# koszullab/chromosight

Hardware: AMD Instinct MI355X
Metric: Mpixels/s normxcorr2 (17x17 loops kernel) (higher is better)
Workload: dtype f32

## Files before the change

chromosight_amd/csrc/cs_corr_mfma.hip:

```cpp
#include "cs_device.h"
#include <algorithm>
#include <cstdlib>
#include <cstring>
#include <mutex>
#include <utility>
#include <vector>

#include "cs_launch.h"

namespace cs {

typedef _Float16 h8 __attribute__((ext_vector_type(8)));

__device__ __forceinline__ float cand_range_guard(float r, float s2, float unscale, const KernelStats<float>& K);
typedef _Float16 h4 __attribute__((ext_vector_type(4)));
typedef float f4 __attribute__((ext_vector_type(4)));
typedef float f4u __attribute__((ext_vector_type(4), aligned(4)));
typedef double d2u __attribute__((ext_vector_type(2), aligned(8)));

constexpr int MF_T = 64;
constexpr int MF_R = 80;
constexpr int MF_PLANE = MF_R * MF_R * 2;
constexpr int MF_WSET = 17 * 2 * 1024;
constexpr int MF_SCR_PITCH = 40;
// ... 226 lines not shown

    load_set(0);
    __syncthreads();
    MF_STAMP(3);
    for (int s = 0; s < km; ++s) {
        const h8 bh = reinterpret_cast<const h8*>(wreg)[(2 * s + 0) * 64 + lane];
        const h8 bl = reinterpret_cast<const h8*>(wreg)[(2 * s + 1) * 64 + lane];
#pragma unroll
        for (int c = 0; c < 4; ++c) {
            const int off = (wr0 + s + n) * MF_R + 16 * c + 8 * g;
            const h8 ah = *reinterpret_cast<const h8*>(xh + off);
            const h8 al = *reinterpret_cast<const h8*>(xl + off);
            accM[c] = mfma16(ah, bh, accM[c]);
            accC[c] = mfma16(ah, bl, accC[c]);
            accC[c] = mfma16(al, bh, accC[c]);
        }
    }
    MF_STAMP(4);
    if constexpr (MASKED) {
        for (int set = 1; set <= 2; ++set) {
            __syncthreads();
            load_set(set);
            __syncthreads();
            for (int s = 0; s < km; ++s) {
                const h8 bh = reinterpret_cast<const h8*>(wreg)[(2 * s + 0) * 64 + lane];
                const h8 bl = reinterpret_cast<const h8*>(wreg)[(2 * s + 1) * 64 + lane];
#pragma unroll
                for (int c = 0; c < 4; ++c) {
                    const int off = (wr0 + s + n) * MF_R + 16 * c + 8 * g;
                    const h8 am = *reinterpret_cast<const h8*>(xm + off);
                    if (set == 1) {
                        KA[c] = mfma16(am, bh, KA[c]);
                        KA[c] = mfma16(am, bl, KA[c]);
                    } else {
                        KB[c] = mfma16(am, bh, KB[c]);
                        KB[c] = mfma16(am, bl, KB[c]);
                    }
                }
            }
        }
    }

    MF_STAMP(5);
    const float u_cs = unscale * E.unscale[0];
    const float u_s2 = 32.0f * unscale;
#pragma unroll
    for (int c = 0; c < 4; ++c) {
        const int j = J0 + 16 * c + n;
#pragma unroll
        for (int v = 0; v < 4; ++v) {
            const int i = I0 + wr0 + 4 * g + v;
            if (i >= A.row_end || j < 0 || j >= A.ns) continue;
            const int d = j - i;
            if (d < A.out_lo || d > A.out_hi) continue;
            const float cs = (accM[c][v] + accC[c][v]) * u_cs;
            const float s1 = S1[c][v] * unscale;
            const float s2 = (S2[c][v] * u_s2) * unscale;
            float r, nobs = A.ks.n;
            if (pixel_forced_zero(A, i, j)) {
                r = 0.0f;
            } else if (A.xcorr_only) {
                r = (fabsf(cs) < A.ks.thr) ? 0.0f : cs;
            } else if constexpr (MASKED) {
                const float nm = NM[c][v];
                const float ka = KA[c][v] * E.unscale[1], kb = KB[c][v] * E.unscale[2];
                r = cand_range_guard(pearson_masked_lean(cs, s1, s2, nm, ka, kb, A.ks), s2, unscale, A.ks);
                nobs = A.ks.n - nm;
            } else {
                r = cand_range_guard(pearson_nomask_lean(cs, s1, s2, A.ks), s2, unscale, A.ks);
            }
            store_pixel(A, i, j, r, nobs);
        }
    }
    MF_STAMP(6);
}

#ifdef CS_MF_PROFILE
extern "C" int cs_debug_mfma_profile(unsigned long long* out)
{
    hipError_t e = hipMemcpyFromSymbol(out, HIP_SYMBOL(cs_mf_prof), sizeof(cs_mf_prof));
    if (e != hipSuccess) return (int)e;
    unsigned long long zero[16] = {0};
    return (int)hipMemcpyToSymbol(HIP_SYMBOL(cs_mf_prof), zero, sizeof(zero));
}
#endif

struct MfmaFixArgs {
    int fix_on, fix_hi_w, fix_hi_d0;
    const float* fix_lo;
    const float* fix_hi;
    const float* fix_rows;
    const float* fix_cols;
    int fix_top, fix_bot0, fix_width, fix_xband, fix_xlo, fix_side;
    const float* rim;
    int max_dist;
};

struct MfmaDenseArgs {
    const float* sig;
    void* out;
    int out_is_f64;
    long long ld_in, ld_out, row0_in, row0_out;
    int ms, ns, km, kn;
    int row_begin, row_end;
    int full, sym_upper;
    int xcorr_only;
    int tiles_x, n_tiles;
    int by_cut;
    const uint4* frag;
    float w_unscale;
    float wa_unscale, wb_unscale;
    int xcd_order;
    int dbg;
    KernelStats<float> ks;
    int band_in, lo_in, bw_in;
    int pad_in;
    int cnt_in;
    int band_out, lo_out;
    int out_lo, out_hi;
    float* nobs;
    const float* w;
    const uint8_t* miss_col;
    const float* rowtab;
    const float* coltab;
    int fix_on, fix_hi_w, fix_hi_d0, fix_top, fix_bot0, fix_any_side;
    int rim_in_kernel;
    MfmaFixArgs fx;
};

constexpr int MFD_ROWS_PER_THREAD = 14;
constexpr int MFD_WL = 4 * MF_PLANE;
constexpr int MFD_SCR = MFD_WL + 18 * 1024;
constexpr int MFD_RED = MFD_SCR + 4 * 2 * MF_SCR_PLANE;
constexpr int MFD_SMEM = MFD_RED + 64;
constexpr int MFD_COL = MFD_RED + 64;
constexpr int MFD_CFL = MFD_COL + 2 * 3 * 64 * 4;
constexpr int MFD_CFB = MFD_CFL + 2 * 16;
constexpr int MFD_SMEM_REG = MFD_CFB + 2 * 128;
static_assert(MFD_SMEM_REG <= 80 * 1024, "two workgroups per CU");
#ifdef CS_MF_PROFILE
constexpr int MFD_PROF = MFD_SMEM_REG;
constexpr int MFD_LAUNCH_EXTRA = 128;
#else
constexpr int MFD_LAUNCH_EXTRA = 0;
#endif

__device__ __forceinline__ unsigned pack_h2(_Float16 a, _Float16 b)
{
    typedef _Float16 h2 __attribute__((ext_vector_type(2)));
    h2 v;
    v[0] = a;
    v[1] = b;
    return __builtin_bit_cast(unsigned, v);
}

__device__ __forceinline__ void lds_barrier()
{
    __builtin_amdgcn_fence(__ATOMIC_RELEASE, "workgroup", "local");
    __builtin_amdgcn_s_waitcnt(0xc07f);
    __builtin_amdgcn_s_barrier();
    __builtin_amdgcn_fence(__ATOMIC_ACQUIRE, "workgroup", "local");
}

__device__ __forceinline__ float wave_max_nonneg(float v)
{
#define CS_DPP_MAX(ctrl, rmask)                                                                                  \
    v = fmaxf(v, __builtin_bit_cast(float, __builtin_amdgcn_update_dpp(0, __builtin_bit_cast(int, v), ctrl, rmask, 0xf, true)))
    CS_DPP_MAX(0x111, 0xf);
    CS_DPP_MAX(0x112, 0xf);
    CS_DPP_MAX(0x114, 0xf);
    CS_DPP_MAX(0x118, 0xf);
    CS_DPP_MAX(0x142, 0xa);
    CS_DPP_MAX(0x143, 0xc);
#undef CS_DPP_MAX
    return v;
}

__device__ __forceinline__ void wave_lds_sync()
{
    __builtin_amdgcn_fence(__ATOMIC_RELEASE, "wavefront");
    __builtin_amdgcn_wave_barrier();
    __builtin_amdgcn_fence(__ATOMIC_ACQUIRE, "wavefront");
}

__device__ __forceinline__ float cand_range_guard(float r, float s2, float unscale, const KernelStats<float>& K)
{
    if (K.cand_cmin > 0.0f) r = ((int)(s2 > 0.0f) & (int)(s2 < K.n * (unscale * unscale) * 0.0625f)) ? 2.0f : r;
    return r;
}

__device__ __attribute__((noinline)) float masked_coefficient_rare(float cs, float s1, float s2, float nm, float ka, float kb,
                                                                   const KernelStats<float>& K)
{
    return pearson_masked_f32(cs, s1, s2, nm, ka, kb, K);
}

__device__ __forceinline__ float masked_coefficient(float cs, float s1, float s2, float nm, float ka, float kb,
                                                    const KernelStats<float>& K)
{
    bool rare;
    float r = pearson_masked_core(cs, s1, s2, nm, ka, kb, K, rare);
    if (rare) r = masked_coefficient_rare(cs, s1, s2, nm, ka, kb, K);
    return r;
}

typedef const __attribute__((address_space(4))) MfmaFixArgs* FixArgsPtr;

__device__ __forceinline__ FixArgsPtr fix_args()
{
    unsigned long long kv = (unsigned long long)__builtin_amdgcn_kernarg_segment_ptr();
    asm volatile("" : "+s"(kv));
    return (FixArgsPtr)(kv + offsetof(MfmaDenseArgs, fx));
}

typedef const __attribute__((address_space(4))) KernelStats<float>* StatsPtr;

__device__ __forceinline__ StatsPtr stats_args()
{
    unsigned long long kv = (unsigned long long)__builtin_amdgcn_kernarg_segment_ptr();
    asm volatile("" : "+s"(kv));
    return (StatsPtr)(kv + offsetof(MfmaDenseArgs, ks));
}

typedef const __attribute__((address_space(4))) MfmaDenseArgs* ArgsPtr;

__device__ __forceinline__ ArgsPtr args_here()
{
    unsigned long long kv = (unsigned long long)__builtin_amdgcn_kernarg_segment_ptr();
    asm volatile("" : "+s"(kv));
    return (ArgsPtr)kv;
}

typedef const __attribute__((address_space(4))) CountsHeader* CountsHdrPtr;

__device__ __forceinline__ CountsHdrPtr counts_header(const float* band)
{
    return (CountsHdrPtr)((unsigned long long)band - (unsigned long long)kCountsHeaderBytes);
}

__device__ __forceinline__ ArgsPtr args_at(unsigned long long entry)
{
    asm volatile("" : "+s"(entry));
    return (ArgsPtr)entry;
}

__device__ __forceinline__ FixArgsPtr fix_args_at(unsigned long long entry)
{
    asm volatile("" : "+s"(entry));
    return (FixArgsPtr)(entry + offsetof(MfmaDenseArgs, fx));
}

__device__ __forceinline__ StatsPtr stats_args_at(unsigned long long entry)
{
    asm volatile("" : "+s"(entry));
    return (StatsPtr)(entry + offsetof(MfmaDenseArgs, ks));
}

template <typename AT>
__device__ __forceinline__ const float* mask_fix_record(AT& A, FixArgsPtr F, int i, int j)
{
    const int K = A.km, KH = (A.km - 1) / 2;
    const int d = j - i;
    const int fix_on = F->fix_on, fix_side = F->fix_side, fix_top = F->fix_top, fix_bot0 = F->fix_bot0, fix_hi_d0 = F->fix_hi_d0,
              fix_hi_w = F->fix_hi_w;
    const float* fix_cols = F->fix_cols;
    const bool in_range = (j >= 0) & (j < A.ns) & (d >= A.out_lo) & (d <= A.out_hi) & (i < A.row_end);
    const int x = F->fix_xband ? d - F->fix_xlo : j;
    const bool top = i < fix_top;
    const bool bot = (i >= fix_bot0) & (!fix_on | (i + KH >= A.ms) | (j + KH >= A.ns));
    const bool side = (fix_cols != nullptr) & ((j < fix_side) | (j >= A.ns - fix_side));
    const bool edge_rec = (fix_on != 0) & (A.rim_in_kernel == 0);
    const bool lo = edge_rec & (d >= 0) & (d < K - 1);
    const bool hi = edge_rec & (d >= fix_hi_d0) & (d - fix_hi_d0 < fix_hi_w);
    const long long o_rows = (long long)(top ? i : fix_top + i - fix_bot0) * F->fix_width + x;
    const long long o_side = (long long)i * 2 * fix_side + (j < fix_side ? j : j - (A.ns - 2 * fix_side));
    const long long o_lo = (long long)i * (K - 1) + d;
    const long long o_hi = (long long)i * fix_hi_w + (d - fix_hi_d0);
    const float* base = (top | bot) ? F->fix_rows : side ? fix_cols : lo ? F->fix_lo : F->fix_hi;
    const long long off = (top | bot) ? o_rows : side ? o_side : lo ? o_lo : o_hi;
    return (in_range & (top | bot | side | lo | hi)) ? base + 4 * off : nullptr;
}

__device__ __forceinline__ void rim_correction(const float* __restrict__ T, int K, int D, int md, unsigned rbits, unsigned cbits,
                                               float& fn, float& fa, float& fb)
{
    fn = fa = fb = 0.0f;
    if (D < K - 1) {
        fn = T[kRimBase + D];
        fa = T[kRimBase + 17 + D];
        fb = T[kRimBase + 34 + D];
    }
    for (unsigned rb = rbits; rb; rb &= rb - 1) {
        const int ki = __builtin_ctz(rb);
        const int L = min(K, max(0, ki - D));
        const int H = min(K, max(0, md - D + ki + 1));
        const float* pa = T + kRimPW + ki * 18;
        const float* pb = pa + 17 * 18;
        fn -= (float)(L + (K - H));
        fa -= pa[L] + (pa[K] - pa[H]);
        fb -= pb[L] + (pb[K] - pb[H]);
    }
    for (unsigned cb = cbits; cb; cb &= cb - 1) {
        const int kj = __builtin_ctz(cb);
        const int lo_k = min(K, max(0, kj + D + 1));
        const int hi_k = min(K, max(0, kj - (md - D)));
        const float* qa = T + kRimQW + kj * 18;
// ... 381 lines not shown
```

chromosight_amd/csrc/cs_corr_mfma_body.inc:

```

    extern __shared__ __attribute__((aligned(16))) char smem[];
    char* const pl_xh = smem;
    char* const pl_xl = smem + MF_PLANE;
    char* const pl_qh = smem + 2 * MF_PLANE;
    char* const pl_ql = smem + 3 * MF_PLANE;
    float* const raw = reinterpret_cast<float*>(smem + 2 * MF_PLANE);
    const int tid = threadIdx.x;
    const int lane = tid & 63, wv = tid >> 6;
    const int n = lane & 15, g = lane >> 4;
    char* const scr = smem + MFD_SCR + wv * (2 * MF_SCR_PLANE);
    unsigned* const red = reinterpret_cast<unsigned*>(smem + MFD_RED);
    const int km = A.km, kn = A.kn;
    const int kh = (km - 1) / 2, kw = (kn - 1) / 2;
#ifdef CS_MF_PROFILE
#undef MF_PROF_ADD
#define MF_PROF_ADD(k, v) (prof_lds[k] += (unsigned long long)(v))
    unsigned long long* const prof_lds = reinterpret_cast<unsigned long long*>(smem + MFD_PROF);
    unsigned long long tprev_ = 0;
    if (tid == 0)
        for (int k = 0; k < 16; ++k) prof_lds[k] = 0;
    auto prof_flush = [&]() {
        if (tid == 0)
            for (int k = 0; k < 16; ++k)
                if (prof_lds[k]) atomicAdd(&cs_mf_prof[k], prof_lds[k]);
    };
#endif

    h8 ones_b, ones_p;
#pragma unroll
    for (int e = 0; e < 8; ++e) {
        const int t = 8 * g + e - n;
        ones_b[e] = (t >= 0 && t < kn) ? (_Float16)1.0f : (_Float16)0.0f;
        const int rho = (e < 4 ? 4 * g + e : 16 + 4 * g + (e - 4)) - n;
        ones_p[e] = (rho >= 0 && rho < km) ? (_Float16)1.0f : (_Float16)0.0f;
    }
    const f4 zero4 = {0.0f, 0.0f, 0.0f, 0.0f};
    const int wr0 = 16 * wv;
    const int c2 = tid % 40, rg = tid / 40;
    const int c2_ = c2, rg_ = rg;
    const bool stager = tid < 240;
    const int p_min = max(0, A.row_begin - kh), p_max = min(A.ms, A.row_end + (km - 1) - kh) - 1;
    int pad_row0 = 0x7fffffff;
    if constexpr (REG && VEC4) pad_row0 = A.pad_in ? max(p_min, (int)A.row0_in + 1) : 0x7fffffff;
    float cnt_max = 0.0f;
    const float* cnt_wt = nullptr;
    const float* cnt_rlaw = nullptr;
    int cnt_n = 1, cnt_nd = 1;
    if constexpr (REG && VEC4) {
        if (A.cnt_in) {
            const CountsHdrPtr H = counts_header(A.sig);
            cnt_max = (float)H->max_val;
            cnt_wt = H->weight32;
            cnt_rlaw = H->rlaw32;
            cnt_n = H->n;
            cnt_nd = H->n_diags;
        }
    }

    auto tile_origin = [&](int tile, int& I0, int& J0) {
        if constexpr (LIST) tile = tile_list[tile];
        int by = tile / A.tiles_x;
        int bx = tile - by * A.tiles_x;
        if constexpr (REG) {
            if (by >= A.by_cut) {
                int t = tile - A.by_cut * A.tiles_x;
                by = A.by_cut;
                for (;;) {
                    const int left = A.ns - (A.row_begin + by * MF_T + A.out_lo);
                    const int v = min(A.tiles_x, left <= 0 ? 0 : (left + MF_T - 1) / MF_T);
                    if (t < v) break;
                    t -= v;
                    ++by;
                }
                bx = t;
            }
        }
        I0 = A.row_begin + by * MF_T;
        if constexpr (!REG) {
            const int skew = A.xcd_order >> 1;
            if (skew) {
                bx += (by * skew) % A.tiles_x;
                bx -= bx >= A.tiles_x ? A.tiles_x : 0;
            }
        }
        J0 = bx * MF_T;
        if (REG && A.band_out) J0 += I0 + A.out_lo;
    };
    const int wv_u = __builtin_amdgcn_readfirstlane(wv);
    auto fetch_args = [&]() {
        if constexpr (REG) return TABLE ? args_at(table_entry) : args_here();
        else return &A;
    };
    constexpr int kPiecesPerRow = VEC4 ? MF_R / 4 : MF_R;
    constexpr int kTransfers = VEC4 ? 25 : 100;
    auto fetch = [&](int tile, int slot) {
        const auto FA = fetch_args();
        int I0, J0;
        tile_origin(tile, I0, J0);
        const int P0 = I0 - kh, Q0 = J0 - kw;
        const bool pad_tile = REG && VEC4 && P0 >= pad_row0 && P0 + MF_R - 1 <= p_max;
        int lane_f = lane;
        if constexpr (REG) asm volatile("" : "+v"(lane_f));
        const int e0 = 64 * wv_u + lane_f;
        int r = e0 / kPiecesPerRow, c = e0 - r * kPiecesPerRow;
        if (REG && !MFD_DBG(16384)) {
            if (wv_u < 3) {
                const float* src = FA->coltab + (size_t)wv_u * FA->ns + min(max(J0 + lane_f, 0), FA->ns - 1);
                __builtin_amdgcn_global_load_lds(src, (__attribute__((address_space(3))) void*)(
                    (__attribute__((address_space(3))) char*)(smem) + MFD_COL + (slot * 3 + wv_u) * 256), 4, 0, 0);
            } else {
                const long long base = (long long)(uintptr_t)FA->miss_col;
                const long long first = ((base + Q0) >> 2) << 2;
                long long addr = first + 4 * min(lane_f, 23);
                addr = min(max(addr, (base >> 2) << 2), ((base + FA->ns - 1) >> 2) << 2);
                if (lane_f < 24)
                    __builtin_amdgcn_global_load_lds(reinterpret_cast<const unsigned*>((uintptr_t)addr),
                                                     (__attribute__((address_space(3))) void*)(
                                                         (__attribute__((address_space(3))) char*)(smem) + MFD_CFB + slot * 128), 4, 0, 0);
            }
        }
        if constexpr (REG && VEC4) {
            if (FA->cnt_in) {
                const float* wt = cnt_wt;
                const float* rlaw = cnt_rlaw;
                const int hn = cnt_n, hd = cnt_nd;
#pragma unroll 1
                for (int x = wv_u; x < 5; x += 4) {
                    const int e = 64 * x + lane_f;
                    const bool is_w = e < 160;
                    const int idx = e < 80 ? P0 + e : e < 160 ? Q0 + (e - 80) : Q0 - P0 - (MF_R - 1) + (e - 160);
                    const float* src = (is_w ? wt : rlaw) + min(max(idx, is_w ? 0 : -1), is_w ? hn - 1 : hd);
                    __builtin_amdgcn_global_load_lds(src, (__attribute__((address_space(3))) void*)(
                                                              (__attribute__((address_space(3))) char*)(smem) + MFD_SCR + 256 * x), 4, 0, 0);
                }
            }
        }
        const __attribute__((address_space(3))) char* dst =
            (const __attribute__((address_space(3))) char*)(raw) + (VEC4 ? 1024 : 256) * wv_u;
        if constexpr (REG && VEC4) {
            if (FA->band_in && P0 >= p_min && P0 + MF_R - 1 <= p_max && Q0 - (P0 + MF_R - 1) - FA->lo_in >= 0 &&
                Q0 + MF_R - 1 - P0 - FA->lo_in <= FA->bw_in - 1) {
                const float* src = FA->sig + ((long long)P0 - FA->row0_in) * FA->ld_in + (Q0 - P0 - FA->lo_in) + (long long)r * (FA->ld_in - 1) + 4 * c;
                const long long step_r = 12 * (FA->ld_in - 1) + 64, wrap = (FA->ld_in - 1) - 80;
#pragma unroll 1
                for (int i = wv_u; i < kTransfers; i += 4) {
                    __builtin_amdgcn_global_load_lds(src, (__attribute__((address_space(3))) void*)dst, 16, 0, 0);
                    dst += 4096;
                    c += 16;
                    src += step_r;
                    if (c >= kPiecesPerRow) {
                        c -= kPiecesPerRow;
                        src += wrap;
                    }
                }
                return;
            }
        }
#pragma unroll 1
        for (int i = wv_u; i < kTransfers; i += 4) {
            const int p = min(max(P0 + r, p_min), p_max);
            const float* row = FA->sig + ((long long)p - FA->row0_in) * FA->ld_in;
            if constexpr (VEC4) {
                int q = Q0 + 4 * c;
                if (REG && FA->band_in) q = pad_tile ? min(max(q - p - FA->lo_in, -4), FA->bw_in) : min(max(q - p - FA->lo_in, 0), FA->bw_in - 4);
                else q = min(max(q, 0), FA->ns - 4);
                __builtin_amdgcn_global_load_lds(row + q, (__attribute__((address_space(3))) void*)dst, 16, 0, 0);
                dst += 4096;
                c += 256 % kPiecesPerRow;
                r += 256 / kPiecesPerRow;
            } else {
                int q = min(max(Q0 + c, 0), FA->ns - 1);
                if (REG && FA->band_in) q = min(max(q - p - FA->lo_in, 0), FA->bw_in - 1);
                __builtin_amdgcn_global_load_lds(row + q, (__attribute__((address_space(3))) void*)dst, 4, 0, 0);
                dst += 1024;
                c += 256 % kPiecesPerRow;
                r += 256 / kPiecesPerRow;
            }
            if (c >= kPiecesPerRow) {
                c -= kPiecesPerRow;
                r += 1;
            }
        }
    };

    auto emit = [&](int I0, int J0, float unscale, const f4 (&acc)[4], const f4 (&S1)[4], const f4 (&S2)[4],
                    const f4& hdr, int slot) {
        const float u_cs = unscale * A.w_unscale;
        const float u_s2 = 32.0f * unscale;
        if constexpr (REG) {
            const ArgsPtr EA = TABLE ? args_at(table_entry) : args_here();
            const int K = km;
            const int i = I0 + wr0 + n;
            KernelStats<float> KS;
            {
                const StatsPtr sp = TABLE ? stats_args_at(table_entry) : stats_args();
                KS.n = sp->n; KS.inv_n = sp->inv_n; KS.kmean = sp->kmean; KS.kstd = sp->kstd; KS.kvar = sp->kvar;
                KS.ksum = sp->ksum; KS.k2sum = sp->k2sum; KS.thr = sp->thr; KS.eps = sp->eps; KS.cut = sp->cut;
                KS.thr_n = sp->thr_n; KS.nkvar = sp->nkvar; KS.eps2 = sp->eps2; KS.den2_min = sp->den2_min;
                KS.zk_possible = sp->zk_possible; KS.snap_possible = sp->snap_possible;
                KS.cand_cmin = CAND ? sp->cand_cmin : 0.0f;
                KS.cand_thr = CAND ? sp->cand_thr : 0.0f;
            }
            const float* colb = reinterpret_cast<const float*>(smem + MFD_COL) + slot * 3 * 64;
            const float nr = hdr[0], ra = hdr[1], rb = hdr[2];
            const unsigned* cfm = reinterpret_cast<const unsigned*>(smem + MFD_CFL) + slot * 4;
            const unsigned m0 = __builtin_amdgcn_readfirstlane(cfm[0]), m1 = __builtin_amdgcn_readfirstlane(cfm[1]),
                           m2 = __builtin_amdgcn_readfirstlane(cfm[2]);
            const bool tile_flags = (m0 | m1 | m2) != 0;
            const unsigned row_bits = (tile_flags && !MFD_DBG(128)) ? (unsigned)hdr[3] : 0u;
            const bool cross_on = __builtin_amdgcn_ballot_w64(row_bits != 0) != 0;
            h8 ua_h, ua_t, ub_h, ub_t;
            if (cross_on) {
                float ua[8], ub[8];
#pragma unroll
                for (int e = 0; e < 8; ++e) ua[e] = ub[e] = 0.0f;
                unsigned bits = row_bits;
                while (__builtin_amdgcn_ballot_w64(bits != 0)) {
                    if (bits) {
                        const int ki = __builtin_ctz(bits);
                        bits &= bits - 1;
                        const float* wa = EA->w + K * K + ki * K;
                        const float* wb = EA->w + 2 * K * K + ki * K;
#pragma unroll
                        for (int e = 0; e < 8; ++e) {
                            const int kj = 8 * g + e;
                            const float in = kj < K ? 1.0f : 0.0f;
                            ua[e] = fmaf(wa[min(kj, K - 1)], in, ua[e]);
                            ub[e] = fmaf(wb[min(kj, K - 1)], in, ub[e]);
                        }
                    }
                }
                const float sa = __builtin_amdgcn_rcpf(EA->wa_unscale), sb = __builtin_amdgcn_rcpf(EA->wb_unscale);
#pragma unroll
                for (int e = 0; e < 8; ++e) {
                    const float a = ua[e] * sa, b = ub[e] * sb;
                    ua_h[e] = (_Float16)a;
                    ua_t[e] = (_Float16)(a - (float)ua_h[e]);
                    ub_h[e] = (_Float16)b;
                    ub_t[e] = (_Float16)(b - (float)ub_h[e]);
                }
            }
            MF_STAMP(7);
            const unsigned kmask8 = (((1u << K) - 1u) >> (8 * g)) & 0xffu;
            const int dmin = J0 - (I0 + MF_T - 1), dmax = J0 + MF_T - 1 - I0;
            const bool on_edge_diag = EA->fix_on && ((dmin < K - 1 && dmax >= 0) | (dmax >= EA->fix_hi_d0 && dmin < EA->fix_hi_d0 + EA->fix_hi_w));
            const bool right_or_bottom = !EA->fix_on | (I0 + MF_T - 1 + (K - 1) / 2 >= EA->ms) | (J0 + MF_T - 1 + (K - 1) / 2 >= EA->ns);
            const bool needs_fix = !MFD_DBG(256) && ((I0 < EA->fix_top) | ((I0 + MF_T - 1 >= EA->fix_bot0) & right_or_bottom) | (EA->fix_any_side != 0) |
                                   (on_edge_diag && !EA->rim_in_kernel));
            const bool needs_rim = RSYM && !MFD_DBG(256) && on_edge_diag && EA->rim_in_kernel;
            const bool plain_out = I0 + MF_T <= EA->row_end && J0 >= 0 && J0 + MF_T <= EA->ns && dmin >= EA->out_lo && dmax <= EA->out_hi;
            float* tb = reinterpret_cast<float*>(scr);
            const bool tile_forced = EA->sym_upper && dmin + (kn - km) < 0;
            f4 fxn = zero4, fxa = zero4, fxb = zero4;
            unsigned fxc = 0xffffu;
            if constexpr (RSYM) if (needs_rim) {
                const FixArgsPtr F = TABLE ? fix_args_at(table_entry) : fix_args();
                const int hi_d0 = F->fix_hi_d0, hi_w = F->fix_hi_w;
                const int iw0 = I0 + wr0;
                const int wd_lo = J0 - iw0 - 15, wd_hi = J0 + MF_T - 1 - iw0;
                const bool low = wd_lo < K - 1 && wd_hi >= 0;
                const bool up = wd_hi >= hi_d0 && wd_lo < hi_d0 + hi_w;
                if (low | up) {
                    const float* rimtab = F->rim;
                    const int md = F->max_dist, bot0 = F->fix_bot0;
                    const int KHf = (K - 1) / 2;
                    const int d0 = low ? 0 : hi_d0, dn = low ? K - 1 : hi_w;
                    const int a = i + d0 - J0;
                    const unsigned rb_all = (unsigned)hdr[3];
                    const bool row_ok = (i >= KHf) & (i + KHf < EA->ms) & (i < EA->row_end);
                    fxc = 0u;
#pragma unroll
                    for (int v = 0; v < 4; ++v) {
                        const int c = (a - 4 * g - v + 15) >> 4;
                        const int x = 16 * c + 4 * g + v;
                        const int d = d0 + (x - a), j = J0 + x;
                        const bool framed = (i >= bot0) & ((i + KHf >= EA->ms) | (j + KHf >= EA->ns));
                        const bool on = row_ok & (c >= 0) & (c <= 3) & (x - a < dn) & !framed & (j >= KHf) & (j + KHf < EA->ns) &
                                        (d >= EA->out_lo) & (d <= EA->out_hi);
                        float fn = 0.0f, fa = 0.0f, fb = 0.0f;
                        if (on) {
                            const unsigned lo32 = x < 32 ? m0 : x < 64 ? m1 : m2;
                            const unsigned hi32 = x < 32 ? m1 : x < 64 ? m2 : 0u;
                            const unsigned cb = (unsigned)((((unsigned long long)hi32 << 32) | lo32) >> (x & 31)) & ((1u << K) - 1u);
                            rim_correction(rimtab, K, d, md, rb_all, cb, fn, fa, fb);
                        }
                        fxn[v] = fn;
                        fxa[v] = fa;
                        fxb[v] = fb;
                        fxc |= (on ? (unsigned)c : 15u) << (4 * v);
                    }
                }
// ... 109 lines not shown
                        }
                        bool live = s2 > 0.0f;
                        if (tile_forced) {
                            const bool forced = d + (kn - km) < 0;
                            if (forced) val = 0.0f;
                            live &= !forced;
                        }
                        if (!plain_out) live &= (i < EA->row_end) & (j >= 0) & (j < EA->ns) & (d >= EA->out_lo) & (d <= EA->out_hi);
                        if (rare && live) rare_bits |= 1u << (4 * cc + v);
                        rv[cc][v] = val;
                    }
                }
#pragma unroll 1
                for (int k = 0; k < (CAND ? 0 : 8); ++k) {
                    if (!__builtin_amdgcn_ballot_w64((rare_bits >> k) != 0)) break;
                    if ((rare_bits >> k) & 1u) {
                        float cs = 0.0f, s1 = 0.0f, s2 = 0.0f, nm = 0.0f, ka = 0.0f, kb = 0.0f;
#pragma unroll
                        for (int e = 0; e < 8; ++e) {
                            const int c = 2 * half + (e >> 2), v = e & 3;
                            if (e == k) {
                                cs = acc[c][v] * u_cs;
                                s1 = S1[c][v] * unscale;
                                s2 = (S2[c][v] * u_s2) * unscale;
                                nm = nmv[e >> 2][v];
                                ka = kav[e >> 2][v];
                                kb = kbv[e >> 2][v];
                            }
                        }
                        const float val = pearson_masked_f32(cs, s1, s2, nm, ka, kb, KS);
#pragma unroll
                        for (int e = 0; e < 8; ++e)
                            if (e == k) rv[e >> 2][e & 3] = val;
                    }
                }
                MF_STAMP(10);
                if constexpr (CAND) {
                    unsigned long long* keys = reinterpret_cast<unsigned long long*>(EA->out);
                    unsigned long long* counter = reinterpret_cast<unsigned long long*>(EA->nobs);
                    float top = rv[0][0];
#pragma unroll
                    for (int e = 1; e < 8; ++e) top = fmaxf(top, rv[e >> 2][e & 3]);
                    if (!__builtin_amdgcn_ballot_w64(top >= KS.cand_thr)) continue;
#pragma unroll
                    for (int cc = 0; cc < 2; ++cc) {
#pragma unroll
                        for (int v = 0; v < 4; ++v) {
                            const int j = J0 + 16 * (2 * half + cc) + 4 * g + v;
                            const int d = j - i;
                            const bool hit = (rv[cc][v] >= KS.cand_thr) & (i < EA->row_end) & (j >= 0) & (j < EA->ns) &
                                             (d >= EA->out_lo) & (d <= EA->out_hi);
                            const unsigned long long m = __builtin_amdgcn_ballot_w64(hit);
                            if (m) {
                                const int first = __builtin_ctzll(m);
                                unsigned long long base = 0;
                                if (lane == first) base = atomicAdd(counter, (unsigned long long)__builtin_popcountll(m));
                                const unsigned lo = __builtin_amdgcn_readlane((unsigned)base, first);
                                const unsigned hi = __builtin_amdgcn_readlane((unsigned)(base >> 32), first);
                                const unsigned long long pos = (((unsigned long long)hi << 32) | lo) +
                                                               (unsigned long long)__builtin_popcountll(m & ((1ull << lane) - 1ull));
                                if (hit && pos < (unsigned long long)EA->ld_out)
                                    keys[pos] = (unsigned long long)EA->row0_out + (unsigned long long)i * (unsigned long long)EA->ns + (unsigned long long)j;
                            }
                        }
                    }
                    continue;
                }
                const int pass_n = EA->nobs ? 2 : 1;
                for (int pass = 0; pass < pass_n; ++pass) {
                    wave_lds_sync();
                    f4 t0 = rv[0], t1 = rv[1];
                    if (pass) {
#pragma unroll
                        for (int v = 0; v < 4; ++v) {
                            t0[v] = KS.n - nmv[0][v];
                            t1[v] = KS.n - nmv[1][v];
                        }
                    }
                    *reinterpret_cast<f4*>(tb + n * 36 + 4 * g) = t0;
                    *reinterpret_cast<f4*>(tb + n * 36 + 16 + 4 * g) = t1;
                    wave_lds_sync();
                    if (plain_out) {
                        const int rr = lane >> 3, c4 = 4 * (lane & 7);
                        const f4 lo = *reinterpret_cast<const f4*>(tb + rr * 36 + c4);
                        const f4 hi = *reinterpret_cast<const f4*>(tb + (rr + 8) * 36 + c4);
                        const int oi = I0 + wr0 + rr, oj = J0 + 32 * half + c4;
                        const long long idx = ((long long)oi - EA->row0_out) * EA->ld_out + (EA->band_out ? oj - oi - EA->lo_out : oj);
                        const long long idx8 = idx + 8 * (long long)EA->ld_out - (EA->band_out ? 8 : 0);
                        if (pass == 1) {
                            *reinterpret_cast<f4u*>(EA->nobs + idx) = lo;
                            *reinterpret_cast<f4u*>(EA->nobs + idx8) = hi;
                        } else if (EA->out_is_f64) {
                            double* od = reinterpret_cast<double*>(EA->out);
                            d2u a, b;
                            a[0] = lo[0]; a[1] = lo[1]; b[0] = lo[2]; b[1] = lo[3];
                            *reinterpret_cast<d2u*>(od + idx) = a;
                            *reinterpret_cast<d2u*>(od + idx + 2) = b;
                            a[0] = hi[0]; a[1] = hi[1]; b[0] = hi[2]; b[1] = hi[3];
                            *reinterpret_cast<d2u*>(od + idx8) = a;
                            *reinterpret_cast<d2u*>(od + idx8 + 2) = b;
                        } else {
                            float* of = reinterpret_cast<float*>(EA->out);
                            *reinterpret_cast<f4u*>(of + idx) = lo;
                            *reinterpret_cast<f4u*>(of + idx8) = hi;
                        }
                        continue;
                    }
                    const int rr = lane >> 3, c4 = 4 * (lane & 7);
                    const f4 lo = *reinterpret_cast<const f4*>(tb + rr * 36 + c4);
                    const f4 hi = *reinterpret_cast<const f4*>(tb + (rr + 8) * 36 + c4);
                    const int oj = J0 + 32 * half + c4;
#pragma unroll
                    for (int part = 0; part < 2; ++part) {
                        const int oi = I0 + wr0 + rr + 8 * part;
                        const f4 v4 = part ? hi : lo;
                        const int first = max(oj, max(0, oi + EA->out_lo)), last = min(oj + 3, min(EA->ns - 1, oi + EA->out_hi));
                        const bool row_ok = !MFD_DBG(1) & (oi < EA->row_end);
                        const long long idx = ((long long)oi - EA->row0_out) * EA->ld_out + (EA->band_out ? oj - oi - EA->lo_out : oj);
                        if (row_ok & (first == oj) & (last == oj + 3)) {
                            if (pass == 1) {
                                *reinterpret_cast<f4u*>(EA->nobs + idx) = v4;
                            } else if (EA->out_is_f64) {
                                double* od = reinterpret_cast<double*>(EA->out);
                                d2u a, b;
                                a[0] = v4[0]; a[1] = v4[1]; b[0] = v4[2]; b[1] = v4[3];
                                *reinterpret_cast<d2u*>(od + idx) = a;
                                *reinterpret_cast<d2u*>(od + idx + 2) = b;
                            } else {
                                *reinterpret_cast<f4u*>(reinterpret_cast<float*>(EA->out) + idx) = v4;
                            }
                        } else if (row_ok & (first <= last)) {
#pragma unroll
                            for (int e = 0; e < 4; ++e) {
                                if ((oj + e >= first) & (oj + e <= last)) {
                                    if (pass == 1) EA->nobs[idx + e] = v4[e];
                                    else if (EA->out_is_f64) reinterpret_cast<double*>(EA->out)[idx + e] = (double)v4[e];
                                    else reinterpret_cast<float*>(EA->out)[idx + e] = v4[e];
                                }
                            }
                        }
                    }
                }
                MF_STAMP(11);
            }
            return;
        }
        if constexpr (!TABLE) {
        const bool plain = I0 + MF_T <= A.row_end && J0 + MF_T <= A.ns &&
                           (A.full || (I0 >= kh && I0 + MF_T - 1 <= A.ms - km + kh && J0 >= kw && J0 + MF_T - 1 <= A.ns - kn + kw)) &&
                           (!A.sym_upper || J0 - (I0 + MF_T - 1) + (A.full ? kn - km : 0) >= 0);
        const int i = I0 + wr0 + n;
        const long long o_idx = ((long long)i - A.row0_out) * A.ld_out + (J0 + 4 * g);
        f4 rv[4];
#pragma unroll
        for (int c = 0; c < 4; ++c) {
#pragma unroll
            for (int v = 0; v < 4; ++v) {
                const float cs = acc[c][v] * u_cs;
                const float s1 = S1[c][v] * unscale;
                const float s2 = (S2[c][v] * u_s2) * unscale;
                rv[c][v] = A.xcorr_only ? (fabsf(cs) < A.ks.thr ? 0.0f : cs)
                                        : MFD_DBG(32) ? cs + s1 + s2
                                                       : cand_range_guard(pearson_nomask_lean(cs, s1, s2, MFD_NOMASK_KS), s2, unscale, MFD_NOMASK_KS);
            }
        }
        if MFD_DBG(1) {
            if (rv[0][0] == 123.456f) reinterpret_cast<float*>(A.out)[o_idx] = rv[1][1] + rv[2][2] + rv[3][3];
        } else if (plain && VEC4) {
            float* tb = reinterpret_cast<float*>(scr);
            const long long r_idx = ((long long)(I0 + wr0 + (lane >> 3)) - A.row0_out) * A.ld_out + J0 + 4 * (lane & 7);
#pragma unroll
            for (int half = 0; half < 2; ++half) {
                wave_lds_sync();
                *reinterpret_cast<f4*>(tb + n * 36 + 4 * g) = rv[2 * half];
                *reinterpret_cast<f4*>(tb + n * 36 + 16 + 4 * g) = rv[2 * half + 1];
                wave_lds_sync();
                const f4 lo = *reinterpret_cast<const f4*>(tb + (lane >> 3) * 36 + 4 * (lane & 7));
                const f4 hi = *reinterpret_cast<const f4*>(tb + ((lane >> 3) + 8) * 36 + 4 * (lane & 7));
                if (A.out_is_f64) {
                    typedef double d2 __attribute__((ext_vector_type(2)));
                    double* od = reinterpret_cast<double*>(A.out) + r_idx + 32 * half;
                    d2 a, b;
                    a[0] = lo[0]; a[1] = lo[1]; b[0] = lo[2]; b[1] = lo[3];
                    *reinterpret_cast<d2*>(od) = a;
                    *reinterpret_cast<d2*>(od + 2) = b;
                    a[0] = hi[0]; a[1] = hi[1]; b[0] = hi[2]; b[1] = hi[3];
                    *reinterpret_cast<d2*>(od + 8 * A.ld_out) = a;
                    *reinterpret_cast<d2*>(od + 8 * A.ld_out + 2) = b;
                } else {
                    float* of = reinterpret_cast<float*>(A.out) + r_idx + 32 * half;
                    *reinterpret_cast<f4*>(of) = lo;
                    *reinterpret_cast<f4*>(of + 8 * A.ld_out) = hi;
                }
            }
        } else {
#pragma unroll
            for (int c = 0; c < 4; ++c) {
#pragma unroll
                for (int v = 0; v < 4; ++v) {
                    const int j = J0 + 16 * c + 4 * g + v;
                    bool z = false;
                    if (!A.full) z = (i < kh) | (i > A.ms - km + kh) | (j < kw) | (j > A.ns - kn + kw);
                    if (A.sym_upper) z = z | ((j - i) + (A.full ? (kn - km) : 0) < 0);
                    if (i < A.row_end && j < A.ns) {
                        const float val = z ? 0.0f : rv[c][v];
                        if (A.out_is_f64) reinterpret_cast<double*>(A.out)[o_idx + 16 * c + v] = (double)val;
                        else reinterpret_cast<float*>(A.out)[o_idx + 16 * c + v] = val;
                    }
                }
            }
        }
        }
    };

    f4 p_acc[4], p_S1[4], p_S2[4], p_hdr = zero4;
    int p_I0 = 0, p_J0 = 0, p_slot = 0, slot = 0;
    float p_unscale = 0.0f;
    bool pending = false;
#pragma unroll
    for (int c = 0; c < 4; ++c) p_acc[c] = p_S1[c] = p_S2[c] = zero4;

    int tile, tile_end, tile_step;
    if constexpr (TABLE) {
        tile = table_tile;
        tile_end = table_tile_end;
        tile_step = table_tile_step;
    } else if ((A.xcd_order & 1) && gridDim.x % 8 == 0) {
        const int x = blockIdx.x & 7, per = (A.n_tiles + 7) / 8;
        tile = x * per + (blockIdx.x >> 3);
        tile_end = min(A.n_tiles, (x + 1) * per);
        tile_step = gridDim.x >> 3;
    } else {
        tile = blockIdx.x;
        tile_end = A.n_tiles;
        tile_step = gridDim.x;
    }
    if MFD_DBG(2048) return;
    if (tile < tile_end) fetch(tile, 0);

    constexpr int kHeads = RSYM ? 1 : 17;
    h8 wh[kHeads];
    {
        const h8* frag = reinterpret_cast<const h8*>(A.frag);
        h8 z;
#pragma unroll
        for (int e = 0; e < 8; ++e) z[e] = (_Float16)0.0f;
        if constexpr (!RSYM) {
#pragma unroll
            for (int s = 0; s < kHeads; ++s) {
                const int sc = min(s, km - 1);
                const h8 a = frag[(2 * sc + 0) * 64 + lane];
                wh[s] = s < km ? a : z;
            }
        } else {
            wh[0] = z;
        }
        constexpr int kSlots = RSYM ? 18 : 17;
        h8 tails[5];
#pragma unroll
        for (int k = 0; k < 5; ++k) {
            const int idx = min(tid + 256 * k, kSlots * 64 - 1);
            const int slot = idx >> 6;
            const int row = RSYM ? (slot < 9 ? slot : slot - 9) : slot, part = RSYM ? (slot < 9 ? 1 : 0) : 1;
            tails[k] = frag[(2 * min(row, km - 1) + part) * 64 + (idx & 63)];
        }
#pragma unroll
        for (int k = 0; k < 5; ++k) {
            const int idx = tid + 256 * k;
            const int slot = idx >> 6;
            const int row = RSYM ? (slot < 9 ? slot : slot - 9) : slot;
            if (idx < kSlots * 64) reinterpret_cast<h8*>(smem + MFD_WL)[idx] = row < km ? tails[k] : z;
        }
    }
    for (;; tile += tile_step) {
        const bool have = REG ? tile < tile_end : true;
        if constexpr (REG) {
            if (!have && !pending) break;
        } else {
            if (tile >= tile_end) break;
        }
        int I0 = 0, J0 = 0;
        if (have) tile_origin(tile, I0, J0);
        const int P0 = I0 - kh, Q0 = J0 - kw;
        bool inside = P0 >= p_min && P0 + MF_R - 1 <= p_max && Q0 >= 0 && Q0 + MF_R <= A.ns;
        if (REG && A.band_in) inside = inside && Q0 - (P0 + MF_R - 1) - A.lo_in >= 0 && Q0 + MF_R - 1 - P0 - A.lo_in <= A.bw_in - 1;
        if (REG && VEC4) inside = inside || (P0 >= pad_row0 && P0 + MF_R - 1 <= p_max);
        if (REG && MFD_DBG(512)) inside = true;
        if MFD_DBG(1024) {
            if (!have) break;
            continue;
        }
        float unscale = 0.0f;
#ifdef CS_MF_PROFILE
        tprev_ = __builtin_readcyclecounter();
        if (tid == 0 && have) prof_lds[15] += 1ull;
#endif
        if (have) {

            bool cnt_tile = false;
            if constexpr (REG && VEC4) cnt_tile = A.cnt_in != 0;

            __builtin_amdgcn_s_waitcnt(0x0f70);
            lds_barrier();
            float xa[MFD_ROWS_PER_THREAD], xb[MFD_ROWS_PER_THREAD];
            float amax = 0.0f;
            if (inside) {
// ... 18 lines not shown
                            const int p = P0 + r, q = Q0 + 2 * c2, cs = (2 * c2) & ~3;
                            const int w = A.band_in ? A.bw_in : A.ns;
                            const int off = A.band_in ? p + A.lo_in : 0;
                            const int idx_s = Q0 + cs - off;
                            const int idx_c = min(max(idx_s, 0), w - 4);
                            const int oa = (2 * c2 - cs) + (idx_s - idx_c), ob = oa + 1;
                            const int idx_a = q - off;
                            const bool rok = (p >= p_min) & (p <= p_max);
                            const bool oka = rok & (q >= 0) & (q < A.ns) & (idx_a >= 0) & (idx_a < w) & (oa >= 0) & (oa < 4);
                            const bool okb = rok & (q + 1 >= 0) & (q + 1 < A.ns) & (idx_a + 1 >= 0) & (idx_a + 1 < w) & (ob >= 0) & (ob < 4);
                            const float* piece = raw + r * MF_R + cs;
                            a = oka ? piece[min(max(oa, 0), 3)] : 0.0f;
                            b = okb ? piece[min(max(ob, 0), 3)] : 0.0f;
                        }
                    } else if (stager && r < MF_R) {
                        const float2 v = *reinterpret_cast<const float2*>(raw + r * MF_R + 2 * c2);
                        const int p = P0 + r, q = Q0 + 2 * c2;
                        const bool rok = (p >= p_min) & (p <= p_max);
                        bool oka = rok & (q >= 0) & (q < A.ns), okb = rok & (q + 1 >= 0) & (q + 1 < A.ns);
                        if (REG && A.band_in) {
                            const int dd = q - p - A.lo_in;
                            oka &= (dd >= 0) & (dd < A.bw_in);
                            okb &= (dd + 1 >= 0) & (dd + 1 < A.bw_in);
                        }
                        a = oka ? v.x : 0.0f;
                        b = okb ? v.y : 0.0f;
                    }
                    xa[k] = a;
                    xb[k] = b;
                    amax = fmaxf(amax, fmaxf(fabsf(a), fabsf(b)));
                }
            }
            if (cnt_tile) {
                const float* cwin = reinterpret_cast<const float*>(smem + MFD_SCR);
                int c2 = c2_, rg = rg_;
                asm volatile("" : "+v"(c2), "+v"(rg));
                typedef float f2 __attribute__((ext_vector_type(2)));
                const f2 cw = *reinterpret_cast<const f2*>(cwin + 80 + 2 * c2);
                const float max_f = cnt_max > 0.0f ? cnt_max : __uint_as_float(0x7f800000u);
                float thin_min = __uint_as_float(0x7f800000u);
                float fa[MFD_ROWS_PER_THREAD], fb[MFD_ROWS_PER_THREAD];
                amax = 0.0f;
                const float* wrow = cwin + rg;
                const float* rld = cwin + 160 + (MF_R - 1) + 2 * c2 - rg - 6 * (MFD_ROWS_PER_THREAD - 1);
#pragma unroll
                for (int k = 0; k < MFD_ROWS_PER_THREAD; ++k) {
                    const float rwk = wrow[6 * k];
                    f2 rl;
                    rl[0] = rld[6 * (MFD_ROWS_PER_THREAD - 1 - k)];
                    rl[1] = rld[6 * (MFD_ROWS_PER_THREAD - 1 - k) + 1];
                    f2 x;
                    x[0] = xa[k];
                    x[1] = xb[k];
                    f2 o = ((x * f2{rwk, rwk}) * cw) * rl;
                    const f2 t = o - f2{max_f, max_f};
                    thin_min = fminf(fminf(fabsf(t[0]), fabsf(t[1])), thin_min);
                    float a = fmaxf(o[0], 0.0f), b = fmaxf(o[1], 0.0f);
                    a = a >= max_f ? 1.0f : a;
                    b = b >= max_f ? 1.0f : b;
                    fa[k] = a;
                    fb[k] = b;
                    amax = fmaxf(amax, fmaxf(a, b));
                }
                bool thin_any = __builtin_amdgcn_ballot_w64(thin_min <= max_f * 2e-6f) != 0;
                if (thin_any && cnt_max > 0.0f) {
                    const CountsHdrPtr H = counts_header(A.sig);
                    const int hn = H->n, hd = H->n_diags;
                    const double* wt = H->weight + H->row0;
                    const double* law = H->law;
                    const double* rlaw = H->rlaw;
                    const double max_val = H->max_val;
                    amax = 0.0f;
#pragma unroll 1
                    for (int k = 0; k < MFD_ROWS_PER_THREAD; ++k) {
                        const int r = rg + 6 * k;
                        const int p = P0 + r, q = Q0 + 2 * c2, d = q - p;
                        const double rwk = wt[min(max(p, 0), hn - 1)];
                        float xk = 0.0f, yk = 0.0f;
                        if (stager && r < MF_R) {
                            if (inside) {
                                const float2 v = *reinterpret_cast<const float2*>(raw + r * MF_R + 2 * c2);
                                xk = v.x;
                                yk = v.y;
                            } else {
                                const int cs = (2 * c2) & ~3;
                                const int w = A.band_in ? A.bw_in : A.ns;
                                const int off = A.band_in ? p + A.lo_in : 0;
                                const int idx_s = Q0 + cs - off;
                                const int idx_c = min(max(idx_s, 0), w - 4);
                                const int oa = (2 * c2 - cs) + (idx_s - idx_c), ob = oa + 1;
                                const int idx_a = q - off;
                                const bool rok = (p >= p_min) & (p <= p_max);
                                const bool oka = rok & (q >= 0) & (q < A.ns) & (idx_a >= 0) & (idx_a < w) & (oa >= 0) & (oa < 4);
                                const bool okb = rok & (q + 1 >= 0) & (q + 1 < A.ns) & (idx_a + 1 >= 0) & (idx_a + 1 < w) & (ob >= 0) & (ob < 4);
                                const float* piece = raw + r * MF_R + cs;
                                xk = oka ? piece[min(max(oa, 0), 3)] : 0.0f;
                                yk = okb ? piece[min(max(ob, 0), 3)] : 0.0f;
                            }
                        }
                        const int da = min(max(d, 0), hd - 1), db = min(max(d + 1, 0), hd - 1);
                        const float a = (float)stage_detrend_rcp(((double)xk * rwk) * wt[min(max(q, 0), hn - 1)], rlaw[da], max_val, law + da);
                        const float b = (float)stage_detrend_rcp(((double)yk * rwk) * wt[min(max(q + 1, 0), hn - 1)], rlaw[db], max_val, law + db);
#pragma unroll
                        for (int e = 0; e < MFD_ROWS_PER_THREAD; ++e) {
                            fa[e] = e == k ? a : fa[e];
                            fb[e] = e == k ? b : fb[e];
                        }
                        amax = fmaxf(amax, fmaxf(fabsf(a), fabsf(b)));
                    }
                }
#pragma unroll
                for (int k = 0; k < MFD_ROWS_PER_THREAD; ++k) {
                    xa[k] = fa[k];
                    xb[k] = fb[k];
                }
            }
            amax = wave_max_nonneg(amax);
            if (lane == 63) red[wv] = __float_as_uint(amax);
            if constexpr (REG) {
                if (wv < 2) {
                    const int q = Q0 + tid;
                    const long long start = (long long)(uintptr_t)A.miss_col + Q0;
                    const int skew = (int)(start - ((start >> 2) << 2));
                    const uint8_t fb = reinterpret_cast<const uint8_t*>(smem + MFD_CFB)[slot * 128 + skew + min(tid, 79)];
                    const bool flagged = tid < 80 && q >= 0 && q < A.ns && fb;
                    const unsigned long long m = __builtin_amdgcn_ballot_w64(flagged);
                    unsigned* cfm = reinterpret_cast<unsigned*>(smem + MFD_CFL) + slot * 4;
                    if (lane == 0) {
                        cfm[2 * wv] = (unsigned)m;
                        if (wv == 0) cfm[1] = (unsigned)(m >> 32);
                    }
                }
            }
            MF_STAMP(0);
            lds_barrier();
            int ex = 0;
            {
                const uint4 m4 = *reinterpret_cast<const uint4*>(red);
                const unsigned mx = max(max(m4.x, m4.y), max(m4.z, m4.w));
                const int e = (int)((mx >> 23) & 0xffu);
                if (e != 0 && e != 255) ex = 6 - (e - 127);
                ex = max(-100, min(100, ex));
            }
            const float scale = __uint_as_float((unsigned)(ex + 127) << 23);
            const float qscale = __uint_as_float((unsigned)(ex + 127 - 5) << 23);
            unscale = __uint_as_float((unsigned)(127 - ex) << 23);
            typedef __fp16 hv2 __attribute__((ext_vector_type(2)));
#pragma unroll
            for (int k = 0; k < MFD_ROWS_PER_THREAD; ++k) {
                const int r = rg + 6 * k;
                if (stager && r < MF_R && !MFD_DBG(16)) {
                    const float a = xa[k] * scale, b = xb[k] * scale;
                    const hv2 hh = __builtin_amdgcn_cvt_pkrtz(a, b);
                    const hv2 tt = __builtin_amdgcn_cvt_pkrtz(a - (float)hh[0], b - (float)hh[1]);
                    const float qa = (xa[k] * qscale) * a, qb = (xb[k] * qscale) * b;
                    const hv2 qh = __builtin_amdgcn_cvt_pkrtz(qa, qb);
                    const hv2 qt = __builtin_amdgcn_cvt_pkrtz(qa - (float)qh[0], qb - (float)qh[1]);
                    const int o = (r * MF_R + 2 * c2) * 2;
                    *reinterpret_cast<hv2*>(pl_xh + o) = hh;
                    *reinterpret_cast<hv2*>(pl_xl + o) = tt;
                    *reinterpret_cast<hv2*>(pl_qh + o) = qh;
                    *reinterpret_cast<hv2*>(pl_ql + o) = qt;
                }
            }
            MF_STAMP(1);
        } else if (REG) {
            __builtin_amdgcn_s_waitcnt(0x0f70);
            lds_barrier();
        }
        if (pending) emit(p_I0, p_J0, p_unscale, p_acc, p_S1, p_S2, p_hdr, p_slot);
        if (!have) break;
        MF_STAMP(6);
        lds_barrier();

        f4 S1[4], S2[4];
#pragma unroll
        for (int c = 0; c < 4; ++c) S1[c] = S2[c] = zero4;
        if (!MFD_DBG(4) && !A.xcorr_only) {
            auto hfrag = [&](int t, h8 (&f)[4]) {
                const int c = t >> 1;
                const char* ph = (t & 1) ? pl_qh : pl_xh;
                const char* pt = (t & 1) ? pl_ql : pl_xl;
#pragma unroll
                for (int rb = 0; rb < 2; ++rb) {
                    const int off = ((wr0 + 16 * rb + n) * MF_R + 16 * c + 8 * g) * 2;
                    f[2 * rb] = *reinterpret_cast<const h8*>(ph + off);
                    f[2 * rb + 1] = *reinterpret_cast<const h8*>(pt + off);
                }
            };
            h8 cur[4];
            hfrag(0, cur);
#pragma unroll
            for (int t = 0; t < 8; ++t) {
                h8 nxt[4];
                if (t + 1 < 8) hfrag(t + 1, nxt);
                h8 bh, bl;
#pragma unroll
                for (int rb = 0; rb < 2; ++rb) {
                    f4 h = mfma16(cur[2 * rb], ones_b, zero4);
                    h = mfma16(cur[2 * rb + 1], ones_b, h);
#pragma unroll
                    for (int v = 0; v < 4; ++v) {
                        const _Float16 hh = (_Float16)h[v];
                        bh[4 * rb + v] = hh;
                        bl[4 * rb + v] = (_Float16)(h[v] - (float)hh);
                    }
                }
                f4 sacc = mfma16(bh, ones_p, zero4);
                sacc = mfma16(bl, ones_p, sacc);
                if (t & 1) S2[t >> 1] = sacc;
                else S1[t >> 1] = sacc;
                if (t + 1 < 8) {
#pragma unroll
                    for (int q = 0; q < 4; ++q) cur[q] = nxt[q];
                }
            }
        }
        MF_STAMP(2);
        lds_barrier();
        if (tile + tile_step < tile_end && !MFD_DBG(2)) fetch(tile + tile_step, slot ^ 1);

        MF_STAMP(3);
        f4 acc[4];
#pragma unroll
        for (int c = 0; c < 4; ++c) acc[c] = zero4;
        h8 ah[4], al[4], bl;
        const int fo = ((wr0 + n) * MF_R + 8 * g) * 2;
#pragma unroll
        for (int c = 0; c < 4; ++c) {
            ah[c] = *reinterpret_cast<const h8*>(pl_xh + fo + 32 * c);
            al[c] = *reinterpret_cast<const h8*>(pl_xl + fo + 32 * c);
        }
        h8 bh;
        bl = reinterpret_cast<const h8*>(smem + MFD_WL)[lane];
        if constexpr (RSYM) bh = reinterpret_cast<const h8*>(smem + MFD_WL)[9 * 64 + lane];
        else bh = wh[0];
        if (!MFD_DBG(8))
#pragma unroll
        for (int s = 0; s < 17; ++s) {
            h8 nh[4], nl[4], nb, nbh;
            if (s + 1 < 17) {
#pragma unroll
                for (int c = 0; c < 4; ++c) {
                    nh[c] = *reinterpret_cast<const h8*>(pl_xh + fo + (s + 1) * MF_R * 2 + 32 * c);
                    nl[c] = *reinterpret_cast<const h8*>(pl_xl + fo + (s + 1) * MF_R * 2 + 32 * c);
                }
                const int sn = RSYM && s + 1 > 8 ? 16 - (s + 1) : s + 1;
                nb = reinterpret_cast<const h8*>(smem + MFD_WL)[sn * 64 + lane];
                if constexpr (RSYM) nbh = reinterpret_cast<const h8*>(smem + MFD_WL)[(9 + sn) * 64 + lane];
                else nbh = wh[s + 1];
            }
            __builtin_amdgcn_sched_barrier(0);
#pragma unroll
            for (int c = 0; c < 4; ++c) acc[c] = mfma16(bh, ah[c], acc[c]);
#pragma unroll
            for (int c = 0; c < 4; ++c) acc[c] = mfma16(bl, ah[c], acc[c]);
#pragma unroll
            for (int c = 0; c < 4; ++c) acc[c] = mfma16(bh, al[c], acc[c]);
            __builtin_amdgcn_sched_barrier(0);
            if (s + 1 < 17) {
#pragma unroll
                for (int c = 0; c < 4; ++c) {
                    ah[c] = nh[c];
                    al[c] = nl[c];
                }
                bl = nb;
                bh = nbh;
            }
        }
        MF_STAMP(4);
#pragma unroll
        for (int c = 0; c < 4; ++c) {
            p_acc[c] = acc[c];
            p_S1[c] = S1[c];
            p_S2[c] = S2[c];
        }
        p_I0 = I0;
        p_J0 = J0;
        p_unscale = unscale;
        p_slot = slot;
        if constexpr (REG) p_hdr = *reinterpret_cast<const f4*>(A.rowtab + 4 * (size_t)min(I0 + wr0 + n, A.ms - 1));
        slot ^= 1;
        pending = true;
    }
    if constexpr (!REG) {
        if (pending) emit(p_I0, p_J0, p_unscale, p_acc, p_S1, p_S2, p_hdr, p_slot);
    }
#ifdef CS_MF_PROFILE
    prof_flush();
#undef MF_PROF_ADD
#define MF_PROF_ADD(k, v) atomicAdd(&cs_mf_prof[k], (unsigned long long)(v))
#endif
```

Measured before the change: 188,100.

## Add lean Pearson epilogue, direct async tile fetch, and fused f16 residual split

For the non-REG dense path, tiles are now fetched straight from the input with global_load_lds when the tile lies fully in bounds, skipping the generic staging path. The Pearson epilogue gets a lean fast path using rsq and fmed3 clamping. A per-wave ballot falls back to the guarded pearson/cand_range_guard path whenever any lane's values are near thresholds. The hi/lo f16 splitting uses v_fma_mix to subtract the packed half directly, avoiding separate f16-to-f32 conversions. The risks are slightly different rounding and extra branching and register pressure.

Measured after the change: 208,300 (median of 6 runs). 10.8% higher.

```diff
diff --git a/chromosight_amd/csrc/cs_corr_mfma.hip b/chromosight_amd/csrc/cs_corr_mfma.hip
--- a/chromosight_amd/csrc/cs_corr_mfma.hip
+++ b/chromosight_amd/csrc/cs_corr_mfma.hip
@@ -402,6 +402,20 @@
     v[0] = a;
     v[1] = b;
     return __builtin_bit_cast(unsigned, v);
+}
+
+__device__ __forceinline__ float sub_f16_lo(float x, unsigned h)
+{
+    float r;
+    asm("v_fma_mix_f32 %0, -%1, 1.0, %2 op_sel_hi:[1,0,0]" : "=v"(r) : "v"(h), "v"(x));
+    return r;
+}
+
+__device__ __forceinline__ float sub_f16_hi(float x, unsigned h)
+{
+    float r;
+    asm("v_fma_mix_f32 %0, -%1, 1.0, %2 op_sel:[1,0,0] op_sel_hi:[1,0,0]" : "=v"(r) : "v"(h), "v"(x));
+    return r;
 }
 
 __device__ __forceinline__ void lds_barrier()
diff --git a/chromosight_amd/csrc/cs_corr_mfma_body.inc b/chromosight_amd/csrc/cs_corr_mfma_body.inc
--- a/chromosight_amd/csrc/cs_corr_mfma_body.inc
+++ b/chromosight_amd/csrc/cs_corr_mfma_body.inc
@@ -137,6 +137,24 @@
         }
         const __attribute__((address_space(3))) char* dst =
             (const __attribute__((address_space(3))) char*)(raw) + (VEC4 ? 1024 : 256) * wv_u;
+        if constexpr (!REG && VEC4) {
+            if (P0 >= p_min && P0 + MF_R - 1 <= p_max && Q0 >= 0 && Q0 + MF_R <= FA->ns) {
+                const float* src = FA->sig + ((long long)P0 + r - FA->row0_in) * FA->ld_in + Q0 + 4 * c;
+                const long long step_r = 12 * FA->ld_in + 64, wrap = FA->ld_in - 80;
+#pragma unroll 1
+                for (int i = wv_u; i < kTransfers; i += 4) {
+                    __builtin_amdgcn_global_load_lds(src, (__attribute__((address_space(3))) void*)dst, 16, 0, 0);
+                    dst += 4096;
+                    c += 16;
+                    src += step_r;
+                    if (c >= kPiecesPerRow) {
+                        c -= kPiecesPerRow;
+                        src += wrap;
+                    }
+                }
+                return;
+            }
+        }
         if constexpr (REG && VEC4) {
             if (FA->band_in && P0 >= p_min && P0 + MF_R - 1 <= p_max && Q0 - (P0 + MF_R - 1) - FA->lo_in >= 0 &&
                 Q0 + MF_R - 1 - P0 - FA->lo_in <= FA->bw_in - 1) {
@@ -552,6 +570,35 @@
         const int i = I0 + wr0 + n;
         const long long o_idx = ((long long)i - A.row0_out) * A.ld_out + (J0 + 4 * g);
         f4 rv[4];
+        bool lean = !A.xcorr_only && !MFD_DBG(32) && !(MFD_NOMASK_KS.cand_cmin > 0.0f);
+        if (lean) {
+            const KernelStats<float>& KS = MFD_NOMASK_KS;
+            const float inv_u = __uint_as_float((254u << 23) - __float_as_uint(unscale));
+            const float t1 = KS.thr_n * inv_u;
+            const float t2 = (t1 * inv_u) * 0.03125f;
+            const float td = (KS.den2_min * inv_u) * inv_u;
+            const float top = (fmaxf(KS.kvar, 1.0f) * 4294967296.0f) * (unscale * unscale);
+            auto normal_or_0 = [](float x) { return x == 0.0f || (x >= 1.17549435e-38f && x <= 3.40282347e38f); };
+            lean = normal_or_0(t1) && normal_or_0(t2) && normal_or_0(td) && td > 0.0f && top <= 3.40282347e38f;
+            if (lean) {
+                const float n32 = 32.0f * KS.n, wu = A.w_unscale;
+                bool normal = true;
+#pragma unroll
+                for (int c = 0; c < 4; ++c) {
+#pragma unroll
+                    for (int v = 0; v < 4; ++v) {
+                        const float s1 = S1[c][v], s2 = S2[c][v], cw = acc[c][v] * wu;
+                        const float den2 = fmaf(s2, n32, -s1 * s1) * KS.kvar;
+                        float r = cw * __builtin_amdgcn_rsqf(den2);
+                        r = (den2 >= td) ? r : 0.0f;
+                        rv[c][v] = __builtin_amdgcn_fmed3f(r, -1.0f, 1.0f);
+                        normal &= (int)(fabsf(s1) >= t1) & (int)(s2 >= t2) & (int)(fabsf(fmaf(KS.kmean, s1, cw)) >= t1);
+                    }
+                }
+                lean = !__builtin_amdgcn_ballot_w64(!normal);
+            }
+        }
+        if (!lean)
 #pragma unroll
         for (int c = 0; c < 4; ++c) {
 #pragma unroll
@@ -876,10 +923,17 @@
                 if (stager && r < MF_R && !MFD_DBG(16)) {
                     const float a = xa[k] * scale, b = xb[k] * scale;
                     const hv2 hh = __builtin_amdgcn_cvt_pkrtz(a, b);
-                    const hv2 tt = __builtin_amdgcn_cvt_pkrtz(a - (float)hh[0], b - (float)hh[1]);
                     const float qa = (xa[k] * qscale) * a, qb = (xb[k] * qscale) * b;
                     const hv2 qh = __builtin_amdgcn_cvt_pkrtz(qa, qb);
-                    const hv2 qt = __builtin_amdgcn_cvt_pkrtz(qa - (float)qh[0], qb - (float)qh[1]);
+                    hv2 tt, qt;
+                    if constexpr (!REG) {
+                        const unsigned hu = __builtin_bit_cast(unsigned, hh), qu = __builtin_bit_cast(unsigned, qh);
+                        tt = __builtin_amdgcn_cvt_pkrtz(sub_f16_lo(a, hu), sub_f16_hi(b, hu));
+                        qt = __builtin_amdgcn_cvt_pkrtz(sub_f16_lo(qa, qu), sub_f16_hi(qb, qu));
+                    } else {
+                        tt = __builtin_amdgcn_cvt_pkrtz(a - (float)hh[0], b - (float)hh[1]);
+                        qt = __builtin_amdgcn_cvt_pkrtz(qa - (float)qh[0], qb - (float)qh[1]);
+                    }
                     const int o = (r * MF_R + 2 * c2) * 2;
                     *reinterpret_cast<hv2*>(pl_xh + o) = hh;
                     *reinterpret_cast<hv2*>(pl_xl + o) = tt;
@@ -919,16 +973,31 @@
                 h8 nxt[4];
                 if (t + 1 < 8) hfrag(t + 1, nxt);
                 h8 bh, bl;
+                typedef unsigned u4 __attribute__((ext_vector_type(4)));
+                u4 bhw, blw;
 #pragma unroll
                 for (int rb = 0; rb < 2; ++rb) {
                     f4 h = mfma16(cur[2 * rb], ones_b, zero4);
                     h = mfma16(cur[2 * rb + 1], ones_b, h);
-#pragma unroll
-                    for (int v = 0; v < 4; ++v) {
-                        const _Float16 hh = (_Float16)h[v];
-                        bh[4 * rb + v] = hh;
-                        bl[4 * rb + v] = (_Float16)(h[v] - (float)hh);
-                    }
+                    if constexpr (!REG) {
+#pragma unroll
+                        for (int pr = 0; pr < 2; ++pr) {
+                            const unsigned hp = pack_h2((_Float16)h[2 * pr], (_Float16)h[2 * pr + 1]);
+                            bhw[2 * rb + pr] = hp;
+                            blw[2 * rb + pr] = pack_h2((_Float16)sub_f16_lo(h[2 * pr], hp), (_Float16)sub_f16_hi(h[2 * pr + 1], hp));
+                        }
+                    } else {
+#pragma unroll
+                        for (int v = 0; v < 4; ++v) {
+                            const _Float16 hh = (_Float16)h[v];
+                            bh[4 * rb + v] = hh;
+                            bl[4 * rb + v] = (_Float16)(h[v] - (float)hh);
+                        }
+                    }
+                }
+                if constexpr (!REG) {
+                    bh = __builtin_bit_cast(h8, bhw);
+                    bl = __builtin_bit_cast(h8, blw);
                 }
                 f4 sacc = mfma16(bh, ones_p, zero4);
                 sacc = mfma16(bl, ones_p, sacc);
```
